# tanmaniac/IntroToComputerVision

Hardware: AMD Instinct MI355X
Metric: Mpix/s (LK 5-level pyramid, 1080p pairs) (higher is better)
Workload: dtype f32

## Files before the change

### introtocomputervision_amd/csrc/lk_fused.hip

```cpp
#include "lk_fused.hpp"

#include <cstdio>
#include <cstdlib>
#include <mutex>
#include <utility>
#include <vector>

#include "lk_device.hpp"
#include "lk_window.hpp"

namespace micv {



template <int NT, int V4, int NROWS>
__device__ __forceinline__ void dma_rows(const float *__restrict__ src, int istride, float *dst, int tid) {
    constexpr int NP = (NROWS * V4 + NT - 1) / NT, A = NT / V4, B = NT % V4;
    const int lane = tid & 63;
    const int slot0 = __builtin_amdgcn_readfirstlane(tid - lane);
    int ly = tid / V4, lv = tid - ly * V4;
    size_t goff = (size_t)ly * istride + 4 * lv;
    const size_t step = (size_t)A * istride + 4 * B, carry = (size_t)istride - 4 * V4;
#pragma unroll
    for (int k = 0; k < NP; k++) {
        if (k == NP - 1 ? (ly < NROWS) : true)
            __builtin_amdgcn_global_load_lds((glb_cvoid *)(src + goff), (lds_void *)(dst + 4 * (slot0 + k * NT)), 16,
                                             0, 0);
        if (k + 1 < NP) {
            lv += B;
            const bool c = lv >= V4;
            lv -= c ? V4 : 0;
            ly += A + (c ? 1 : 0);
            goff += step + (c ? carry : 0);
        }
    }
}

template <int NT, int V4, int NROWS, bool ZERO>
__device__ __forceinline__ void dma_rows_clipped(const float *__restrict__ img, int istride, int rows, int cols,
                                                 int gx0, int gy0, float *dst, int tid) {
    constexpr int NP = (NROWS * V4 + NT - 1) / NT, A = NT / V4, B = NT % V4;
    const int lane = tid & 63;
    const int slot0 = __builtin_amdgcn_readfirstlane(tid - lane);
    int ly = tid / V4, lv = tid - ly * V4;
#pragma unroll
    for (int k = 0; k < NP; k++) {
        if (k == NP - 1 ? (ly < NROWS) : true) {
            const int gy = gy0 + ly, gx = gx0 + 4 * lv;
            const bool in = (unsigned)gy < (unsigned)rows && (unsigned)gx < (unsigned)cols;
            if (in)
                __builtin_amdgcn_global_load_lds((glb_cvoid *)(img + (size_t)gy * istride + gx),
                                                 (lds_void *)(dst + 4 * (slot0 + k * NT)), 16, 0, 0);
            else if (ZERO)
                *reinterpret_cast<v4f *>(dst + 4 * (tid + k * NT)) = (v4f){0.f, 0.f, 0.f, 0.f};
        }
        if (k + 1 < NP) {
            lv += B;
            const bool c = lv >= V4;
            lv -= c ? V4 : 0;
            ly += A + (c ? 1 : 0);
        }
    }
}

template <int NT, int RWC, int NROWS>
__device__ __forceinline__ void dma_gather(const float *__restrict__ src, int rstride, int xs, float *dst, int tid) {
    constexpr int PARTS = (RWC + 63) / 64, NWV = NT / 64, RSTEP = NWV / PARTS, NP = (NROWS + RSTEP - 1) / RSTEP;
    static_assert(NWV % PARTS == 0 && RSTEP >= 1, "a wave keeps its part of the row");
    const int lane = tid & 63, wave = __builtin_amdgcn_readfirstlane(tid >> 6);
    const int part = wave % PARTS, col = 64 * part + lane;
    const unsigned voff = (unsigned)(col * xs);
    if (col < RWC) {
#pragma unroll
        for (int k = 0; k < NP; k++) {
            const int row = wave / PARTS + RSTEP * k;
            if (k == NP - 1 ? row < NROWS : true)
                __builtin_amdgcn_global_load_lds((glb_cvoid *)(src + (size_t)row * rstride + voff),
                                                 (lds_void *)(dst + row * RWC + 64 * part), 4, 0, 0);
        }
    }
}

template <int NT, int RWC, int NROWS, bool ZERO>
__device__ __forceinline__ void dma_gather_clipped(const float *__restrict__ img, int rstride, int xs, int rows,
                                                   int cols, int gx0, int gy0, float *dst, int tid) {
    constexpr int PARTS = (RWC + 63) / 64, NWV = NT / 64, RSTEP = NWV / PARTS, NP = (NROWS + RSTEP - 1) / RSTEP;
    static_assert(NWV % PARTS == 0 && RSTEP >= 1, "a wave keeps its part of the row");
    const int lane = tid & 63, wave = __builtin_amdgcn_readfirstlane(tid >> 6);
    const int part = wave % PARTS, col = 64 * part + lane;
    const int gx = gx0 + col;
    const bool col_in = (unsigned)gx < (unsigned)cols;
    const unsigned voff = col_in ? (unsigned)(gx * xs) : 0u;
    if (col < RWC) {
#pragma unroll
        for (int k = 0; k < NP; k++) {
            const int row = wave / PARTS + RSTEP * k;
            if (k == NP - 1 ? row < NROWS : true) {
                const int gy = gy0 + row;
                const bool row_in = (unsigned)gy < (unsigned)rows;
                if (row_in && col_in)
                    __builtin_amdgcn_global_load_lds((glb_cvoid *)(img + (size_t)gy * rstride + voff),
                                                     (lds_void *)(dst + row * RWC + 64 * part), 4, 0, 0);
                else if (ZERO)
                    dst[row * RWC + col] = 0.f;
            }
        }
    }
}

template <typename C>
__device__ __forceinline__ void dma_coarse(const LkLevelArgs &a, int pair, int cx0, int cy0, float *Cf, int tid) {
    constexpr int Q = C::CWP / 4, HPI = 64 / Q, HALF_ROWS = 2 * C::CH, NI = (HALF_ROWS + HPI - 1) / HPI;
    constexpr int NWV = C::NT / 64;
    const int lane = tid & 63, wave = __builtin_amdgcn_readfirstlane(tid >> 6);
    const int hl = lane / Q, q = lane - hl * Q;
    const int fc = a.flow_cols;
    const float *__restrict__ fu = a.flow_u + pair * a.flow_pair + (size_t)cy0 * fc + cx0 + 4 * q;
    const float *__restrict__ fv = a.flow_v + pair * a.flow_pair + (size_t)cy0 * fc + cx0 + 4 * q;
#pragma unroll
    for (int k = 0; k < (NI + NWV - 1) / NWV; k++) {
        const int it = wave + NWV * k;
        const int hr = it * HPI + hl;
        if (it < NI && hl < HPI && hr < HALF_ROWS)
            __builtin_amdgcn_global_load_lds((glb_cvoid *)(((hr & 1) ? fv : fu) + (size_t)(hr >> 1) * fc),
                                             (lds_void *)(Cf + it * HPI * C::CWP), 16, 0, 0);
    }
}

#include "lk_strip.hpp"

struct LkStreamLink {
    const int4 *sched;
    int per_xcd, xcd;
    unsigned *counter;
    int *slot;
    int4 next;
    bool next_staged;
    float ou[8], ov[8];
};

template <typename C>
__device__ __forceinline__ bool lk_tile_interior(const LkLevelArgs &a, int tile_x, int tile_y) {
    constexpr int E = C::M > 2 ? C::M : 2;
    const int rx0 = tile_x * C::TW - C::H, ry0 = tile_y * C::TH - C::H;
    return rx0 - E >= 0 && rx0 + C::RW + E <= a.cols && ry0 - E >= 0 && ry0 + C::RH + E <= a.rows;
}

template <typename C>
__device__ __forceinline__ void lk_stage_ahead(const LkLevelArgs &a, float *lds, int tile_x, int tile_y, int pair,
                                               int tid) {
    float *Xs = lds + C::IMG_F;
    const int rx0 = tile_x * C::TW - C::H, ry0 = tile_y * C::TH - C::H;
    const int cx0 = (rx0 - 2 > 0 ? rx0 - 2 : 0) >> 1, cy0 = (ry0 - 2 > 0 ? ry0 - 2 : 0) >> 1;
    dma_coarse<C>(a, pair, cx0, cy0, Xs, tid);
    const float *next = a.next + pair * a.img_pair;
    dma_rows<C::NT, C::NW / 4, C::NH>(next + (size_t)(ry0 - C::M) * a.img_stride + rx0 - C::M, a.img_stride,
                                      Xs + C::CS_F, tid);
}

template <int R, int MODE, bool INT, int NTV, bool CARRY = false, int THV = 32, bool STREAM = false,
          bool IN_LOOP = CARRY || STREAM, bool GATHER = false, bool PARTIAL_COLS = false, int TWV = 64, bool PRE = false>
__device__ __forceinline__ void lk_tile(const LkLevelArgs &a, const TapsN<2 * R + 1> &g,
                                        float *lds, int tile_x, int tile_y, int pair, bool more = false,
                                        LkStreamLink *link = nullptr) {
    using C = LkCfg<R, NTV, THV, TWV>;
    constexpr int RPT = C::RPT;
    constexpr int TW = C::TW, TH = C::TH, H = C::H, RW = C::RW, RH = C::RH, PS = C::PS;
    static_assert(TWV == 64 || (!CARRY && !STREAM && !GATHER), "32-wide tiles: the plain kernel only");
    constexpr int GW = C::GW, GH = C::GH, GS = C::GS, GP = C::GP, CW = C::CW, NT = C::NT;
    constexpr int M = C::M, NW = C::NW;
    static_assert(!CARRY || (INT && C::FAST && MODE == LK_FLOW_COARSE && C::CHAIN_OK), "carry tiles: interior, coarse flow");
    static_assert(!STREAM || (INT && C::FAST && MODE == LK_FLOW_COARSE && !CARRY && C::RW % 4 == 0 && C::NW % 4 == 0 && !GATHER),
                  "streamed tiles: interior, coarse flow, LDS-DMA staging");
    static_assert(!(STREAM || (INT && C::FAST && MODE == LK_FLOW_COARSE && !CARRY)) || C::CS_F + C::NW * C::NH <= C::X_F,
                  "interior tiles: DMA-staged coarse block + next window fit the gradient area");
    constexpr int LY0 = CARRY ? C::LYC : 0;
    constexpr int Q0 = CARRY ? C::QC : 0;
    constexpr int CH = CARRY ? C::CHC : C::CH;
    constexpr int NH = CARRY ? C::NHC : C::NH;
    constexpr bool CDMA = STREAM || (INT && C::FAST && MODE == LK_FLOW_COARSE && !CARRY);
    constexpr int CBF = CDMA ? C::CS_F : (CARRY ? C::CC_F : C::C_F);
    constexpr bool STAGED = INT && C::FAST && MODE != LK_FLOW_NONE;
#ifdef MICV_LK_DEFER_PREV
    constexpr bool DEFER = INT && C::FAST && MODE == LK_FLOW_COARSE && !CARRY && !STREAM && !GATHER;
#else
    constexpr bool DEFER = false;
#endif
    const bool fastb = !INT && C::FAST && MODE != LK_FLOW_NONE && a.rows >= 4 && a.cols >= 4;
    float *P = lds;
    float *Wp = lds + RH * PS;
    float *X = lds + C::IMG_F;
    float *Xs = X + (CARRY ? C::CARRY_F : 0);
    v2f *Cuv = reinterpret_cast<v2f *>(Xs);
    float *Ru = Xs + CBF, *Rv = Ru + CH * RW;
    float *Nx = Xs + CBF;
    float *Gx = X, *Gy = X + GP, *Gt = X + 2 * GP;
    float *rb0 = lds, *rb1 = lds + GH * C::RBS, *rb2 = lds + 2 * GH * C::RBS;

    int tid_ = threadIdx.x;
    if (IN_LOOP) asm volatile("" : "+v"(tid_));
    const int tid = tid_;
    const int rows = a.rows, cols = a.cols;
    const int x0 = tile_x * TW, y0 = tile_y * TH + a.y_shift;
    const int rx0 = x0 - H, ry0 = y0 - H;
    const float *__restrict__ prev = a.prev + pair * a.img_pair;
    const float *__restrict__ next = a.next + pair * a.img_pair;
    const int istride = a.img_stride;
    const int xs = GATHER ? a.img_xstride : 1;
    const float g5[5] = {0.0625f, 0.25f, 0.375f, 0.25f, 0.0625f};
#ifdef MICV_DIAG
    const bool stamp_wave = a.stamps != nullptr && __builtin_amdgcn_readfirstlane(tid) < 64;
    unsigned long long t_prev = 0;
    if (stamp_wave) t_prev = __builtin_amdgcn_s_memtime();
#define MICV_STAMP(k)                                                        \
    if (stamp_wave) {                                                        \
        const unsigned long long t_now = __builtin_amdgcn_s_memtime();       \
        if (tid == 0) atomicAdd(&a.stamps[(k) + (INT ? 0 : 8)], t_now - t_prev); \
        t_prev = t_now;                                                      \
    }                                                                        \
    if (a.stop_after == (k)) return;
#define MICV_STOP(k) if (a.stop_after == (k)) return;
#else
#define MICV_STAMP(k)
#define MICV_STOP(k)
#endif

    int cx0 = 0, cy0 = 0;
    constexpr int NC = CDMA ? 1 : (CH * CW + NT - 1) / NT;
    float rcu[NC], rcv[NC];
    if (CDMA) {
        cx0 = (rx0 - 2 > 0 ? rx0 - 2 : 0) >> 1;
        cy0 = (ry0 - 2 > 0 ? ry0 - 2 : 0) >> 1;
        if (!STREAM) dma_coarse<C>(a, pair, cx0, cy0, Xs, tid);
    } else if (MODE == LK_FLOW_COARSE) {
        const float *__restrict__ fu = a.flow_u + pair * a.flow_pair;
        const float *__restrict__ fv = a.flow_v + pair * a.flow_pair;
        const int fr = a.flow_rows, fc = a.flow_cols;
        cx0 = (rx0 - 2 > 0 ? rx0 - 2 : 0) >> 1;
        cy0 = (ry0 + (CARRY ? H : 0) - 2 > 0 ? ry0 + (CARRY ? H : 0) - 2 : 0) >> 1;
        if (fastb) {
            cx0 = (rx0 - 2) >> 1;
            cy0 = (ry0 - 2) >> 1;
        }
#pragma unroll
        for (int k = 0; k < NC; k++) {
            const int i = tid + k * NT < CH * CW ? tid + k * NT : CH * CW - 1;
            const int cy = i / CW, cx = i - cy * CW;
            const int yy = clampi(cy0 + cy, 0, fr - 1), xx = clampi(cx0 + cx, 0, fc - 1);
            rcu[k] = fu[(size_t)yy * fc + xx];
            rcv[k] = fv[(size_t)yy * fc + xx];
        }
    }
    const bool vec_ok = STREAM || GATHER ||
                        (INT && (istride & 3) == 0 && ((a.img_pair & 3) == 0) &&
                         ((reinterpret_cast<uintptr_t>(a.prev) | reinterpret_cast<uintptr_t>(a.next)) & 15) == 0);
    constexpr bool DMA_OK = (RW % 4 == 0) && (NW % 4 == 0);
    bool deferred = false;
    if (INT && DMA_OK && vec_ok) {
        constexpr int V = RW / 4;
        if constexpr (GATHER) {
            if (STAGED)
                dma_gather<NT, NW, NH>(next + (ptrdiff_t)(ry0 - M + LY0) * istride + (ptrdiff_t)(rx0 - M) * xs, istride, xs, Nx, tid);
            dma_gather<NT, RW, RH - LY0>(prev + (size_t)(ry0 + LY0) * istride + (size_t)rx0 * xs, istride, xs, P + LY0 * RW, tid);
            if (MODE == LK_FLOW_NONE)
                dma_gather<NT, RW, RH - LY0>(next + (size_t)(ry0 + LY0) * istride + (size_t)rx0 * xs, istride, xs, Wp + LY0 * RW, tid);
        } else if constexpr (DEFER) {
            dma_rows<NT, NW / 4, NH>(next + (size_t)(ry0 - M + LY0) * istride + rx0 - M, istride, Nx, tid);
            dma_rows<NT, V, RH - LY0>(prev + (size_t)(ry0 + LY0) * istride + rx0, istride, P + LY0 * RW, tid);
            deferred = true;
        } else {
        dma_rows<NT, V, RH - LY0>(prev + (size_t)(ry0 + LY0) * istride + rx0, istride, P + LY0 * RW, tid);
        if (MODE == LK_FLOW_NONE)
            dma_rows<NT, V, RH - LY0>(next + (size_t)(ry0 + LY0) * istride + rx0, istride, Wp + LY0 * RW, tid);
        if (STAGED && !STREAM)
            dma_rows<NT, NW / 4, NH>(next + (size_t)(ry0 - M + LY0) * istride + rx0 - M, istride, Nx, tid);
        }
        if (MODE == LK_FLOW_COARSE && !CDMA) {
#pragma unroll
            for (int k = 0; k < NC; k++) {
                const int i = tid + k * NT;
                if (i < CH * CW) {
                    Cuv[i] = (v2f){rcu[k], rcv[k]};
                }
            }
        }
    } else {
        if (MODE == LK_FLOW_COARSE && !CDMA) {
#pragma unroll
            for (int k = 0; k < NC; k++) {
                const int i = tid + k * NT;
                if (i < CH * CW) {
                    Cuv[i] = (v2f){rcu[k], rcv[k]};
                }
            }
        }
        const bool clip_dma = fastb && (GATHER || ((cols & 3) == 0 && (istride & 3) == 0 && ((a.img_pair & 3) == 0) &&
                              ((reinterpret_cast<uintptr_t>(a.prev) | reinterpret_cast<uintptr_t>(a.next)) & 15) == 0));
        if (GATHER && clip_dma) {
            dma_gather_clipped<NT, NW, NH, true>(next, istride, xs, rows, cols, rx0 - M, ry0 - M, Nx, tid);
            dma_gather_clipped<NT, RW, RH, false>(prev, istride, xs, rows, cols, rx0, ry0, P, tid);
        } else if (clip_dma) {
            dma_rows_clipped<NT, RW / 4, RH, false>(prev, istride, rows, cols, rx0, ry0, P, tid);
            dma_rows_clipped<NT, NW / 4, NH, true>(next, istride, rows, cols, rx0 - M, ry0 - M, Nx, tid);
        } else
        {
            constexpr int NB = (RH * RW + NT - 1) / NT;
            float rp[NB], rn[NB];
#pragma unroll
            for (int k = 0; k < NB; k++) {
                const int i = tid + k * NT < RH * RW ? tid + k * NT : RH * RW - 1;
                const int ly = i / RW, lx = i - ly * RW;
                const int gy = clampi(ry0 + ly, 0, rows - 1), gx = clampi(rx0 + lx, 0, cols - 1);
                rp[k] = prev[(size_t)gy * istride + (size_t)gx * xs];
                if (MODE == LK_FLOW_NONE) rn[k] = next[(size_t)gy * istride + (size_t)gx * xs];
            }
#pragma unroll
            for (int k = 0; k < NB; k++) {
                const int i = tid + k * NT;
                if (i < RH * RW) {
                    P[i] = rp[k];
                    if (MODE == LK_FLOW_NONE) Wp[i] = rn[k];
                }
            }
        }
        if (STAGED) {
            for (int i = tid; i < NH * NW; i += NT) {
                const int ly = i / NW, lx = i - ly * NW;
                Nx[i] = next[(ptrdiff_t)(ry0 - M + LY0 + ly) * istride + (ptrdiff_t)(rx0 - M + lx) * xs];
            }
        }
        if (fastb && !clip_dma) {
            constexpr int NBN = (NH * NW + NT - 1) / NT, HB = (NBN + 1) / 2, A = NT / NW, B = NT % NW;
            int ly = tid / NW, lx = tid - ly * NW;
#pragma unroll
            for (int half = 0; half < 2; half++) {
                float rn[HB];
                int ly2 = ly, lx2 = lx;
#pragma unroll
                for (int k = 0; k < HB; k++) {
                    const int gy = ry0 - M + ly2, gx = rx0 - M + lx2;
                    const bool ok = (unsigned)gy < (unsigned)rows && (unsigned)gx < (unsigned)cols;
                    const float val = next[(size_t)clampi(gy, 0, rows - 1) * istride + (size_t)clampi(gx, 0, cols - 1) * xs];
                    rn[k] = ok ? val : 0.f;
                    lx2 += B;
                    const bool c = lx2 >= NW;
                    lx2 -= c ? NW : 0;
                    ly2 += A + (c ? 1 : 0);
                }
#pragma unroll
                for (int k = 0; k < HB; k++) {
                    const int i = tid + (half * HB + k) * NT;
                    if (i < NH * NW) Nx[i] = rn[k];
                }
                ly = ly2;
                lx = lx2;
            }
        }
    }
    float base_u[RPT], base_v[RPT];
#pragma unroll
    for (int j = 0; j < RPT; j++) base_u[j] = base_v[j] = 0.f;
    if (MODE == LK_FLOW_NONE && a.base_rmw) {
        const int c_ = threadIdx.x & (TW - 1), r0_ = RPT * (threadIdx.x / TW);
#pragma unroll
        for (int j = 0; j < RPT; j++) {
            const int gy = y0 + r0_ + j, gx = x0 + c_;
            if (gy < rows && gx < cols) {
                base_u[j] = a.out_u[pair * a.out_pair + (size_t)gy * a.out_stride + gx];
                base_v[j] = a.out_v[pair * a.out_pair + (size_t)gy * a.out_stride + gx];
            }
        }
    }
    if constexpr (DEFER) {
        if (deferred) {
            constexpr int V = RW / 4, TOT = (RH - LY0) * V, NPP = (TOT + NT - 1) / NT;
            static_assert(NPP >= 1 && NPP <= 8, "prev transfers per wave");
            const bool last = __builtin_amdgcn_readfirstlane(tid) + (NPP - 1) * NT < TOT;
            if (last) {
                asm volatile("s_waitcnt vmcnt(%0)" ::"n"(NPP) : "memory");
            } else {
                asm volatile("s_waitcnt vmcnt(%0)" ::"n"(NPP - 1) : "memory");
            }
            __builtin_amdgcn_s_barrier();
            asm volatile("" ::: "memory");
        } else {
            __syncthreads();
        }
    } else if (MODE != LK_FLOW_NONE && !STREAM) __syncthreads();
    MICV_STAMP(0)

    if (MODE != LK_FLOW_NONE) {
        if (C::FAST && (INT || fastb)) {
            int nx0s = rx0 - M, ny0s = ry0 - M + LY0;
            asm("" : "+s"(nx0s), "+s"(ny0s));
            auto march = [&](int lx, int ly0, float *bu8, float *bv8) {
                const int gx = rx0 + lx, gy0 = ry0 + ly0;
                const float xf32 = 32.f * (float)gx, yf32 = 32.f * (float)gy0;
                typedef __attribute__((address_space(3))) float lds_float;
                lds_float *wrow = (lds_float *)(Wp + ly0 * PS + lx);
                asm("" : "+v"(wrow));
                v2f ruv[RPT / 2 + 2];
                if (MODE == LK_FLOW_COARSE) {
                    const int cyb = ((gy0 >> 1) - 1) - cy0;
                    const int ccb = ((gx >> 1) - 1) - cx0;
                    const int odd = gx & 1;
                    const bool first_col = !INT && gx == 0, last_col = !INT && gx == cols - 1;
                    constexpr int NR = RPT / 2 + 2;
                    v2f cc[CDMA ? 5 * NR : 1];
                    if constexpr (CDMA)
                        coarse_block_load<C>(cc, Xs + cyb * (2 * C::CWP) + ccb, odd, std::make_integer_sequence<int, NR>{});
#pragma unroll
                    for (int i = 0; i < NR; i++) {
                        v2f c0, c1, c2, ca, cb;
                        if constexpr (CDMA) {
                            c0 = cc[5 * i], c1 = cc[5 * i + 1], c2 = cc[5 * i + 2], ca = cc[5 * i + 3], cb = cc[5 * i + 4];
                        } else {
                            const v2f *c = Cuv + (cyb + i) * CW + ccb;
                            c0 = c[0];
                            c1 = c[1];
                            c2 = c[2];
                            ca = c[odd];
                            cb = c[1 + odd];
                        }
                        const v2f t0 = first_col ? c2 : c0, t4 = last_col ? c0 : c2;
                        v2f t = t0 * (v2f){g5[0], g5[0]};
                        t = __builtin_elementwise_fma(ca, (v2f){g5[1], g5[1]}, t);
                        t = __builtin_elementwise_fma(c1, (v2f){g5[2], g5[2]}, t);
                        t = __builtin_elementwise_fma(cb, (v2f){g5[3], g5[3]}, t);
                        ruv[i] = __builtin_elementwise_fma(t4, (v2f){g5[4], g5[4]}, t);
                    }
                }
                float fu_[RPT], fv_[RPT];
                if (MODE == LK_FLOW_FULL) {
#pragma unroll
                    for (int j = 0; j < RPT; j++) {
                        const size_t fo = pair * a.flow_pair + (size_t)(INT ? gy0 + j : clampi(gy0 + j, 0, rows - 1)) * a.flow_cols +
                                          (INT ? gx : clampi(gx, 0, cols - 1));
                        fu_[j] = a.flow_u[fo];
                        fv_[j] = a.flow_v[fo];
                    }
                }
#pragma unroll
                for (int p = 0; p < RPT / 2; p++) {
#pragma unroll
                    for (int o = 0; o < 2; o++) {
                        const int j = 2 * p + o;
                        float bu, bv;
                        v2f half_uv;
                        if (MODE == LK_FLOW_COARSE) {
                            const int i1 = o ? p + 1 : p, i3 = o ? p + 2 : p + 1;
                            v2f ra = ruv[p], rc = ruv[p + 2];
                            if (!INT) asm("" : "+v"(ra), "+v"(rc));
                            const v2f r0 = (!INT && gy0 + j == 0) ? rc : ra;
                            const v2f r4 = (!INT && gy0 + j == rows - 1) ? ra : rc;
                            v2f auv = r0 * (v2f){g5[0], g5[0]};
                            auv = __builtin_elementwise_fma(ruv[i1], (v2f){g5[1], g5[1]}, auv);
                            auv = __builtin_elementwise_fma(ruv[p + 1], (v2f){g5[2], g5[2]}, auv);
                            auv = __builtin_elementwise_fma(ruv[i3], (v2f){g5[3], g5[3]}, auv);
                            auv = __builtin_elementwise_fma(r4, (v2f){g5[4], g5[4]}, auv);
                            half_uv = auv;
                            auv = auv * (v2f){2.f, 2.f};
                            bu = auv.x;
                            bv = auv.y;
                        } else {
                            bu = fu_[j];
                            bv = fv_[j];
                            half_uv = (v2f){bu, bv};
                        }
                        bu8[j] = bu;
                        bv8[j] = bv;
                        if constexpr (DEFER) {
                            if (deferred) {
                                const float wv = warp_sample_staged<NW, NH, 64, true>(
                                    Nx, nx0s, ny0s, next, rows, cols, istride, (v2f){xf32, yf32 + 32.f * (float)j}, half_uv, xs);
                                asm volatile("ds_write_b32 %0, %1 offset:%2" ::"v"(wrow), "v"(wv), "n"(4 * j * PS) : "memory");
                            } else {
                                wrow[j * PS] = warp_sample_staged<NW, NH, 64>(
                                    Nx, nx0s, ny0s, next, rows, cols, istride, (v2f){xf32, yf32 + 32.f * (float)j}, half_uv, xs);
                            }
                        } else if (!CARRY || ly0 + j >= LY0)
                            wrow[j * PS] = warp_sample_staged<NW, NH, MODE == LK_FLOW_COARSE ? 64 : 32>(
                                Nx, nx0s, ny0s, next, rows, cols, istride, (v2f){xf32, yf32 + 32.f * (float)j}, half_uv, xs);
                        if (NT >= 512) __builtin_amdgcn_sched_barrier(0);
                    }
                }
            };
            march(H + (tid & (TW - 1)), H + RPT * (tid / TW), base_u, base_v);
            constexpr int BS = H / RPT, NB = CARRY ? BS : 2 * BS;
            constexpr int SEG0 = CARRY ? (LY0 - H) / RPT : 0, NJ = NB * RW + 2 * H * (TH / RPT - SEG0);
            static_assert(!CARRY || (LY0 >= H && LY0 < H + TH), "carry rows start inside the tile's own rows");
            for (int n = tid; n < (PRE && a.pre_warp ? 0 : NJ); n += NT) {
                int lx, ly0;
                if (n < NB * RW) {
                    const int band = n / RW + (CARRY ? BS : 0);
                    lx = n - (band - (CARRY ? BS : 0)) * RW;
                    ly0 = band < BS ? band * RPT : H + TH + (band - BS) * RPT;
                } else {
                    const int m = n - NB * RW;
                    const int seg = m / (2 * H) + SEG0, cc = m - (seg - SEG0) * (2 * H);
                    lx = cc < H ? cc : TW + cc;
                    ly0 = H + RPT * seg;
                }
                float tu[RPT], tv[RPT];
                march(lx, ly0, tu, tv);
            }
        } else {
            if (MODE == LK_FLOW_COARSE) {
                const int fr = a.flow_rows;
                for (int i = tid; i < CH * RW; i += NT) {
                    const int cy = i / RW, lx = i - cy * RW;
                    const int gx = rx0 + lx;
                    if ((INT || (unsigned)gx < (unsigned)cols) && cy0 + cy < fr) {
                        float au = 0.f, av = 0.f;
#pragma unroll
                        for (int k = 0; k < 5; k++) {
                            const int sc = ((INT ? gx + k - 2 : reflect101(gx + k - 2, cols)) >> 1) - cx0;
                            const v2f cuv = Cuv[cy * CW + sc];
                            au = fmaf(cuv.x, g5[k], au);
                            av = fmaf(cuv.y, g5[k], av);
                        }
                        Ru[i] = au;
                        Rv[i] = av;
                    }
                }
                __syncthreads();
                MICV_STAMP(1)
            }
            auto do_px = [&](int ly, int lx, float &bu, float &bv) {
                const int gy = ry0 + ly, gx = rx0 + lx;
                if (!INT && ((unsigned)gy >= (unsigned)rows || (unsigned)gx >= (unsigned)cols)) return;
                if (MODE == LK_FLOW_COARSE) {
                    float au = 0.f, av = 0.f;
#pragma unroll
                    for (int k = 0; k < 5; k++) {
                        const int rr = ((INT ? gy + k - 2 : reflect101(gy + k - 2, rows)) >> 1) - cy0;
                        au = fmaf(Ru[rr * RW + lx], g5[k], au);
                        av = fmaf(Rv[rr * RW + lx], g5[k], av);
                    }
                    bu = au * 2.f;
                    bv = av * 2.f;
                } else {
                    bu = a.flow_u[pair * a.flow_pair + (size_t)gy * a.flow_cols + gx];
                    bv = a.flow_v[pair * a.flow_pair + (size_t)gy * a.flow_cols + gx];
                }
                Wp[ly * PS + lx] = warp_sample(next, rows, cols, istride, gx, gy, bu, bv, xs);
            };
            {
                const int c = tid & (TW - 1), grp = tid / TW;
#pragma unroll
                for (int j = 0; j < RPT; j++) do_px(H + RPT * grp + j, H + c, base_u[j], base_v[j]);
            }
            constexpr int NHALO = 2 * H * RW + TH * 2 * H;
            for (int n = tid; n < NHALO; n += NT) {
                int ly, lx;
                if (n < 2 * H * RW) {
                    ly = n / RW;
                    lx = n - ly * RW;
                    if (ly >= H) ly += TH;
                } else {
                    const int m = n - 2 * H * RW;
                    const int rr = m / (2 * H), cc = m - rr * (2 * H);
                    ly = H + rr;
                    lx = cc < H ? cc : TW + cc;
                }
                float du_, dv_;
                do_px(ly, lx, du_, dv_);
            }
        }
    }
    if constexpr (DEFER) {
        if (deferred) asm volatile("s_waitcnt vmcnt(0) lgkmcnt(0)" ::: "memory");
    }
    __syncthreads();
    MICV_STAMP(2)
    if constexpr (PRE) {
        if (a.pre_warp) {
            const int c = tid & (TW - 1), r0 = RPT * (tid / TW);
            const int gx = x0 + c;
            float *__restrict__ wb = a.grad + pair * a.grad_pair;
            float *__restrict__ ou = a.out_u + pair * a.out_pair;
            float *__restrict__ ov = a.out_v + pair * a.out_pair;
            if (INT || gx < cols) {
#pragma unroll
                for (int j = 0; j < RPT; j++) {
                    const int gy = y0 + r0 + j;
                    if (INT || gy < rows) {
                        wb[(size_t)gy * cols + gx] = Wp[(H + r0 + j) * PS + H + c];
                        ou[(size_t)gy * a.out_stride + gx] = base_u[j];
                        ov[(size_t)gy * a.out_stride + gx] = base_v[j];
                    }
                }
            }
            return;
        }
    }
    int ticket = 0;
    if (STREAM && tid == 0) ticket = (int)atomicAdd(link->counter, 1u);

    {
        const float s1 = 1.f / 9.f, s2 = 2.f * s1;
        if (!INT) {
            for (int n = tid; n < 2 * RW + 2 * RH; n += NT) {
                int ly, lx;
                if (n < 2 * RW) {
                    ly = (n < RW ? -1 : rows) - ry0;
                    lx = n < RW ? n : n - RW;
                } else {
                    const int m = n - 2 * RW;
                    lx = (m < RH ? -1 : cols) - rx0;
                    ly = m < RH ? m : m - RH;
                }
                if ((unsigned)ly >= (unsigned)RH || (unsigned)lx >= (unsigned)RW) continue;
                const int gy = ry0 + ly, gx = rx0 + lx;
                if (gy >= -1 && gy <= rows && gx >= -1 && gx <= cols) {
                    const int sy = reflect101(gy, rows) - ry0, sx = reflect101(gx, cols) - rx0;
                    if ((unsigned)sy < (unsigned)RH && (unsigned)sx < (unsigned)RW) {
                        P[ly * PS + lx] = P[sy * PS + sx];
                        Wp[ly * PS + lx] = Wp[sy * PS + sx];
                    }
                }
            }
            __syncthreads();
        }
        {
            constexpr int SEG = CARRY ? 6 : (TH == 16 ? 5 : (NT >= 512 ? 4 : 16)), NSEG = (GH - Q0 + SEG - 1) / SEG;
            static_assert(GW % 2 == 0, "gradient columns in pairs");
            constexpr int GW2 = GW / 2;
            const v2f s1v = {s1, s1}, s2v = {s2, s2}, halfv = {0.5f, 0.5f};
            for (int n = tid; n < GW2 * NSEG; n += NT) {
                const int seg = n / GW2, qx = 2 * (n - seg * GW2);
                const int q0 = Q0 + seg * SEG, q1 = q0 + SEG < GH ? q0 + SEG : GH;
                const int lx = qx + (H - R);
                v2f ptx[3], pty[3], wtx[3], wty[3], pcc[3], wcc[3];
                auto rowpass = [&](int ly, int slot) {
                    const float *pr = P + ly * PS + lx, *wr = Wp + ly * PS + lx;
                    v2f pa, pb, pc, wa, wb, wc;
                    if constexpr (((H - R) & 1) == 1 && (PS & 1) == 0) {
                        const v2f p01 = *reinterpret_cast<const v2f *>(pr - 1), p23 = *reinterpret_cast<const v2f *>(pr + 1);
                        const v2f w01 = *reinterpret_cast<const v2f *>(wr - 1), w23 = *reinterpret_cast<const v2f *>(wr + 1);
                        pa = p01; pb = (v2f){p01.y, p23.x}; pc = p23;
                        wa = w01; wb = (v2f){w01.y, w23.x}; wc = w23;
                    } else {
                        pa = (v2f){pr[-1], pr[0]}; pb = (v2f){pr[0], pr[1]}; pc = (v2f){pr[1], pr[2]};
                        wa = (v2f){wr[-1], wr[0]}; wb = (v2f){wr[0], wr[1]}; wc = (v2f){wr[1], wr[2]};
                    }
                    ptx[slot] = pc - pa;
                    pty[slot] = __builtin_elementwise_fma(pc, s1v, __builtin_elementwise_fma(pb, s2v, pa * s1v));
                    wtx[slot] = wc - wa;
                    wty[slot] = __builtin_elementwise_fma(wc, s1v, __builtin_elementwise_fma(wb, s2v, wa * s1v));
                    pcc[slot] = pb;
                    wcc[slot] = wb;
                };
                const int lyb = q0 + (H - R);
                rowpass(lyb - 1, 0);
                rowpass(lyb, 1);
                constexpr int TRIP = SEG <= 6 ? SEG : 3;
#pragma unroll 1
                for (int qy = q0; qy < q1; qy += TRIP) {
#pragma unroll
                    for (int t = 0; t < TRIP; t++) {
                        if (qy + t < q1) {
                            const int s_new = (t + 2) % 3, s_top = t % 3, s_mid = (t + 1) % 3;
                            rowpass(qy + t + (H - R) + 1, s_new);
                            const v2f pgx = __builtin_elementwise_fma(
                                ptx[s_new], s1v, __builtin_elementwise_fma(ptx[s_mid], s2v, ptx[s_top] * s1v));
                            const v2f pgy = pty[s_new] - pty[s_top];
                            const v2f ngx = __builtin_elementwise_fma(
                                wtx[s_new], s1v, __builtin_elementwise_fma(wtx[s_mid], s2v, wtx[s_top] * s1v));
                            const v2f ngy = wty[s_new] - wty[s_top];
                            *reinterpret_cast<v2f *>(Gx + (qy + t) * GS + qx) = ngx * halfv + pgx * halfv;
                            *reinterpret_cast<v2f *>(Gy + (qy + t) * GS + qx) = ngy * halfv + pgy * halfv;
                            *reinterpret_cast<v2f *>(Gt + (qy + t) * GS + qx) = wcc[s_mid] - pcc[s_mid];
                        }
                    }
                }
            }
        }
        if (!INT) {
            __syncthreads();
            auto fill = [&](int qy, int qx) {
                const int gy = y0 - R + qy, gx = x0 - R + qx;
                const int sy = reflect101(gy, rows) - (y0 - R), sx = reflect101(gx, cols) - (x0 - R);
                const bool ok = (unsigned)sy < (unsigned)GH && (unsigned)sx < (unsigned)GW;
                Gx[qy * GS + qx] = ok ? Gx[sy * GS + sx] : 0.f;
                Gy[qy * GS + qx] = ok ? Gy[sy * GS + sx] : 0.f;
                Gt[qy * GS + qx] = ok ? Gt[sy * GS + sx] : 0.f;
            };
            const int rt = clampi(-(y0 - R), 0, GH), rb = clampi(rows - (y0 - R), rt, GH);
            const int cl = clampi(-(x0 - R), 0, GW), cr = clampi(cols - (x0 - R), cl, GW);
            const int n_full = (rt + GH - rb) * GW, side = cl + GW - cr;
            for (int i = tid; i < n_full; i += NT) {
                const int r = i / GW, qx = i - r * GW;
                fill(r < rt ? r : rb + (r - rt), qx);
            }
            if (side > 0) {
                for (int i = tid; i < (rb - rt) * 16; i += NT) {
                    const int qy = rt + (i >> 4);
                    for (int cc = i & 15; cc < side; cc += 16) fill(qy, cc < cl ? cc : cr + (cc - cl));
                }
            }
        }
    }
    __syncthreads();
    MICV_STAMP(3)

    if constexpr (PRE) {
        static_assert(MODE == LK_FLOW_COARSE && !CARRY && !STREAM && TWV == 64, "pre-pass tiles: coarse flow, plain launch");
        const int c = tid & (TW - 1), r0 = RPT * (tid / TW);
        const int gx = x0 + c, pad = a.grad_pad, gp = a.grad_pitch;
        const size_t rowp = 3 * (size_t)gp;
        float *__restrict__ gb = a.grad + pair * a.grad_pair;
        float *__restrict__ ou = a.out_u + pair * a.out_pair;
        float *__restrict__ ov = a.out_v + pair * a.out_pair;
        if (INT || gx < cols) {
            int px2 = -1;
            if (!INT) {
                if (gx >= 1 && gx <= pad) px2 = pad - gx;
                else if (gx >= cols - 1 - pad && gx <= cols - 2) px2 = pad + 2 * (cols - 1) - gx;
            }
#pragma unroll
            for (int j = 0; j < RPT; j++) {
                const int gy = y0 + r0 + j;
                if (INT || gy < rows) {
                    const int q = r0 + j + R, qx = c + R;
                    const float ix = Gx[q * GS + qx], iy = Gy[q * GS + qx], it = Gt[q * GS + qx];
                    auto put = [&](int py, int px) {
                        float *d = gb + (size_t)py * rowp + px;
                        d[0] = ix;
                        d[gp] = iy;
                        d[2 * gp] = it;
                    };
                    put(gy + pad, gx + pad);
                    if (!INT) {
                        int py2 = -1;
                        if (gy >= 1 && gy <= pad) py2 = pad - gy;
                        else if (gy >= rows - 1 - pad && gy <= rows - 2) py2 = pad + 2 * (rows - 1) - gy;
                        if (py2 >= 0) put(py2, gx + pad);
                        if (px2 >= 0) put(gy + pad, px2);
                        if (py2 >= 0 && px2 >= 0) put(py2, px2);
                    }
                    if (a.pre_base) {
                        ou[(size_t)gy * a.out_stride + gx] = base_u[j];
                        ov[(size_t)gy * a.out_stride + gx] = base_v[j];
                    }
                }
            }
        }
        return;
    }

    const int c = tid & (TW - 1), r0 = RPT * (tid / TW);
    float Sxx[RPT], Sxy[RPT], Syy[RPT], Sxt[RPT], Syt[RPT];
    constexpr int RPW = 64 / (TW / 4);
    constexpr int RPI = RPW * (NT / 64);
    constexpr int SWEEP_UNROLL = NT >= 512 ? 1 : 4;
    constexpr int SWEEP_TRIPS = (GH + RPI - 1) / RPI;
    const int sweep_trips = SWEEP_TRIPS == 1 ? 1 + (a.batch < 0 ? 1 : 0) : SWEEP_TRIPS;
    {
        const int lane = tid & 63, wave = tid >> 6;
        const int grp = TW == 64 ? lane >> 2 : ((lane & 3) | ((lane >> 2) & 4)), c0 = 4 * grp;
        const int lrow = TW == 64 ? (lane & 3) : (((lane >> 2) & 3) | ((lane >> 3) & 4));
#pragma unroll SWEEP_UNROLL
        for (int it = 0; it < sweep_trips; it++) {
            const int qy = it * RPI + wave * RPW + lrow;
            if (qy < GH) {
                v2f wx[2 * C::WV], wy[2 * C::WV];
                load_window_pairs<C>(Gx, qy, c0, wx);
                load_window_pairs<C>(Gy, qy, c0, wy);
                const int o = TW == 64 ? rb_off(qy, grp) : rb_off32(qy, grp);
                row_taps_skew<C>(wx, wx, g, rb0 + o);
                if (TH == 16) __builtin_amdgcn_sched_barrier(0);
                row_taps_skew<C>(wx, wy, g, rb1 + o);
                if (TH == 16) __builtin_amdgcn_sched_barrier(0);
                row_taps_skew<C>(wy, wy, g, rb2 + o);
            }
        }
        if (STREAM && tid == 0) *link->slot = ticket;
        __syncthreads();
        MICV_STOP(41)
        int cls[TW == 64 ? 4 : 8];
        if constexpr (TW == 64) {
            col_bases<C>(rb0, c, r0, cls);
            col_pass<C, 0, PARTIAL_COLS>(cls, Sxx, g);
            col_pass<C, 1, PARTIAL_COLS>(cls, Sxy, g);
            col_pass<C, 2, PARTIAL_COLS>(cls, Syy, g);
        } else {
            col_bases32<C>(rb0, c, r0, cls);
            col_pass32<C, 0, PARTIAL_COLS>(cls, Sxx, g);
            col_pass32<C, 1, PARTIAL_COLS>(cls, Sxy, g);
            col_pass32<C, 2, PARTIAL_COLS>(cls, Syy, g);
        }
        if (TH == 16) __builtin_amdgcn_sched_barrier(0);
        __syncthreads();
        MICV_STOP(42)
#pragma unroll SWEEP_UNROLL
        for (int it = 0; it < sweep_trips; it++) {
            const int qy = it * RPI + wave * RPW + lrow;
            if (qy < GH) {
                v2f wx[2 * C::WV], wt[2 * C::WV];
                load_window_pairs<C>(Gx, qy, c0, wx);
                load_window_pairs<C>(Gt, qy, c0, wt);
                const int o = TW == 64 ? rb_off(qy, grp) : rb_off32(qy, grp);
                row_taps_skew<C>(wx, wt, g, rb0 + o);
                if (NT >= 512) __builtin_amdgcn_sched_barrier(0);
                load_window_pairs<C>(Gy, qy, c0, wx);
                row_taps_skew<C>(wx, wt, g, rb1 + o);
            }
        }
        __syncthreads();
        MICV_STOP(43)
        if constexpr (STREAM) {
            const int t = __builtin_amdgcn_readfirstlane(*link->slot);
            link->next = make_int4(0, 0, 0, 0);
            link->next_staged = false;
            if (t < link->per_xcd) {
                const int4 e2 = link->sched[8 * t + link->xcd];
                link->next = e2;
                if (e2.z > 0 && lk_tile_interior<C>(a, e2.x, e2.y)) {
                    lk_stage_ahead<C>(a, lds, e2.x, e2.y, e2.w, tid);
                    link->next_staged = true;
                }
            }
        }
        if (INT && C::CHAIN_OK && MODE == LK_FLOW_COARSE && more) {
            const v4f *src = reinterpret_cast<const v4f *>(X + TH * GS);
            v4f *dst = reinterpret_cast<v4f *>(X);
            for (int i = tid; i < C::CARRY_F / 4; i += NT) dst[i] = src[i];
        }
        if constexpr (TW == 64) {
            col_pass<C, 0, PARTIAL_COLS>(cls, Sxt, g);
            col_pass<C, 1, PARTIAL_COLS>(cls, Syt, g);
        } else {
            col_pass32<C, 0, PARTIAL_COLS>(cls, Sxt, g);
            col_pass32<C, 1, PARTIAL_COLS>(cls, Syt, g);
        }
    }
    MICV_STAMP(4)

    float *__restrict__ ou = a.out_u + pair * a.out_pair;
    float *__restrict__ ov = a.out_v + pair * a.out_pair;
    const int gx = x0 + c;
    if (INT || gx < cols) {
#pragma unroll
        for (int j = 0; j < RPT; j++) {
            const int gy = y0 + r0 + j;
            if (gy >= a.row_begin && gy < a.row_end) {
                float uu, vv;
                lk_solve(Sxx[j], Sxy[j], Syy[j], Sxt[j], Syt[j], uu, vv);
                if (a.add_base) {
                    uu = base_u[j] + uu;
                    vv = base_v[j] + vv;
                }
                if constexpr (STREAM) {
                    link->ou[j] = uu;
                    link->ov[j] = vv;
                } else {
                    ou[(size_t)gy * a.out_stride + gx] = uu;
                    ov[(size_t)gy * a.out_stride + gx] = vv;
                }
            }
        }
    }
    MICV_STAMP(5)
#undef MICV_STAMP
#undef MICV_STOP
}

template <typename C>
__device__ __forceinline__ void lk_tile_of(const LkLevelArgs &a, int bidx, int &tile_x, int &tile_y) {
    constexpr int E = C::M > 2 ? C::M : 2;
    const int nb = gridDim.x, per = nb >> 3, rem = nb & 7;
    const int xcd = bidx & 7, idx = bidx >> 3;
    const int tiles_x = (a.cols + C::TW - 1) / C::TW;
    const int tiles_y = nb / tiles_x, ty_base = a.row_begin / C::TH;
    {
        constexpr int FX = C::TW + C::H + E, FY = C::TH + C::H + E;
        int ix0 = (C::H + E + C::TW - 1) / C::TW, ix1 = a.cols >= FX ? (a.cols - FX) / C::TW + 1 : 0;
        int iy0 = (C::H + E - a.y_shift + C::TH - 1) / C::TH - ty_base;
        int iy1 = (a.rows >= FY + a.y_shift ? (a.rows - FY - a.y_shift) / C::TH + 1 : 0) - ty_base;
        ix1 = ix1 < tiles_x ? ix1 : tiles_x;
        iy0 = iy0 > 0 ? iy0 : 0;
        iy1 = iy1 < tiles_y ? iy1 : tiles_y;
        const int iw = ix1 > ix0 ? ix1 - ix0 : 0, ih = iy1 > iy0 ? iy1 - iy0 : 0;
        const int ni = iw * ih, nbd = nb - ni;
        const int t_plain = xcd * per + (xcd < rem ? xcd : rem) + idx;
        if (ni * 2 >= nb && nb >= 64) {
            const int b0 = (int)(((long long)xcd * nbd) >> 3), b1 = (int)(((long long)(xcd + 1) * nbd) >> 3);
            if (idx < b1 - b0) {
                int b = b0 + idx;
                const int n_top = iy0 * tiles_x, n_bot = (tiles_y - iy1) * tiles_x, side = tiles_x - iw;
                if (b < n_top) {
                    tile_y = b / tiles_x;
                    tile_x = b - tile_y * tiles_x;
                } else if (b < n_top + n_bot) {
                    b -= n_top;
                    tile_y = b / tiles_x;
                    tile_x = b - tile_y * tiles_x;
                    tile_y += iy1;
                } else {
                    b -= n_top + n_bot;
                    const int r = b / side, c = b - r * side;
                    tile_y = iy0 + r;
                    tile_x = c < ix0 ? c : c + iw;
                }
            } else {
                const int i = t_plain - b1;
                const int r = i / iw;
                tile_y = iy0 + r;
                tile_x = ix0 + (i - r * iw);
            }
        } else {
            tile_y = t_plain / tiles_x;
            tile_x = t_plain - tile_y * tiles_x;
        }
        tile_y += ty_base;
    }
}

template <int NT>
__device__ __forceinline__ void lk_build_block(const LkBuildJob &j, int block, int tid) {
    constexpr int RPT = 32 / (NT / 64);
    static_assert(NT % 64 == 0 && 32 % (NT / 64) == 0, "a unit is 32 rows x 64 lanes");
    const int lane = tid & 63, trow = (tid >> 6) * RPT;
    const int l = j.level, rl = j.rows >> l, cl = j.cols >> l;
    const int bx = l == 1 ? (cl + 127) / 128 : (cl + 63) / 64, per_img = bx * ((rl + 31) / 32);
    for (int u = block; u < j.units; u += j.blocks) {
        const int img = u / per_img, r = u - img * per_img;
        const int set = img / j.batch, b = img - set * j.batch;
        const int byi = r / bx, bxi = r - byi * bx;
        const int y0 = byi * 32 + trow;
        const float *src = (set ? j.src_b : j.src_a) + b * j.img_elems;
        float *dst = (set ? j.pyr_b : j.pyr_a) + j.dst_off + (size_t)b * rl * cl;
        if (l == 1) {
            const int x2 = bxi * 64 + lane;
            if (2 * x2 >= cl) continue;
            float4 q[RPT];
#pragma unroll
            for (int i = 0; i < RPT; i++)
                if (y0 + i < rl) q[i] = *reinterpret_cast<const float4 *>(src + (size_t)(2 * (y0 + i) + 1) * j.sstride + 4 * x2);
#pragma unroll
            for (int i = 0; i < RPT; i++)
                if (y0 + i < rl) *reinterpret_cast<float2 *>(dst + (size_t)(y0 + i) * cl + 2 * x2) = make_float2(q[i].y, q[i].w);
        } else {
            const int x = bxi * 64 + lane, sh = (1 << l) - 1;
            if (x >= cl) continue;
            float q[RPT];
#pragma unroll
            for (int i = 0; i < RPT; i++)
                if (y0 + i < rl) q[i] = src[(size_t)(((y0 + i) << l) + sh) * j.sstride + (x << l) + sh];
#pragma unroll
            for (int i = 0; i < RPT; i++)
                if (y0 + i < rl) dst[(size_t)(y0 + i) * cl + x] = q[i];
        }
    }
}

template <int R, int MODE, int NTV, int THV = 32, bool GATHER = false, int TWV = 64>
__global__ __launch_bounds__(NTV, lk_waves_per_simd_rt(R, NTV, THV)) void lk_level_kernel(LkLevelArgs a, TapsN<2 * R + 1> g) {
    using C = LkCfg<R, NTV, THV, TWV>;
    extern __shared__ __attribute__((aligned(16))) float lds[];
    constexpr int E = C::M > 2 ? C::M : 2;
    if (blockIdx.y >= a.batch) {
        lk_build_block<NTV>(a.job, (blockIdx.y - a.batch) * gridDim.x + blockIdx.x, threadIdx.x);
        return;
    }
    int tile_x, tile_y;
    lk_tile_of<C>(a, blockIdx.x, tile_x, tile_y);
    const int rx0 = tile_x * C::TW - C::H, ry0 = tile_y * C::TH + a.y_shift - C::H;
    const bool interior = rx0 - E >= 0 && rx0 + C::RW + E <= a.cols && ry0 - E >= 0 &&
                          ry0 + C::RH + E <= a.rows;
    if (interior)
        lk_tile<R, MODE, true, NTV, false, THV, false, false, GATHER, true, TWV>(a, g, lds, tile_x, tile_y, blockIdx.y);
    else
        lk_tile<R, MODE, false, NTV, false, THV, false, false, GATHER, true, TWV>(a, g, lds, tile_x, tile_y, blockIdx.y);
}

template <int R, int NTV, int THV = 32>
__global__ __launch_bounds__(NTV, lk_waves_per_simd(NTV)) void lk_grad_kernel(LkLevelArgs a) {
    using C = LkCfg<R, NTV, THV>;
    extern __shared__ __attribute__((aligned(16))) float lds[];
    constexpr int E = C::M > 2 ? C::M : 2;
    int tile_x, tile_y;
    lk_tile_of<C>(a, blockIdx.x, tile_x, tile_y);
    const int rx0 = tile_x * C::TW - C::H, ry0 = tile_y * C::TH - C::H;
    const bool interior = rx0 - E >= 0 && rx0 + C::RW + E <= a.cols && ry0 - E >= 0 && ry0 + C::RH + E <= a.rows;
    TapsN<2 * R + 1> g = {};
    if (interior)
        lk_tile<R, LK_FLOW_COARSE, true, NTV, false, THV, false, false, false, false, 64, true>(a, g, lds, tile_x, tile_y, blockIdx.y);
    else
        lk_tile<R, LK_FLOW_COARSE, false, NTV, false, THV, false, false, false, false, 64, true>(a, g, lds, tile_x, tile_y, blockIdx.y);
}

struct LkStripPlan {
    int items, strips, segs, seg_rows;
    int ix0, iw, iy0, ih;
    int tiles_x, tiles_y, border;
};

template <int R, int NTV>
__global__ __launch_bounds__(NTV, lk_waves_per_simd(NTV)) void lk_level_strip_kernel(LkLevelArgs a, TapsN<2 * R + 1> g, LkStripPlan p) {
    using C = LkCfg<R, NTV>;
    extern __shared__ __attribute__((aligned(16))) float lds[];
    int b = blockIdx.x;
    if (b < p.items) {
        const int per = p.items >> 3, rem = p.items & 7;
        const int xcd = b & 7, idx = b >> 3;
        int item = xcd * per + (xcd < rem ? xcd : rem) + idx;
        if (idx >= per + (xcd < rem ? 1 : 0)) return;
        const int strip = item % p.strips, t = item / p.strips;
        const int seg = t % p.segs, pair = t / p.segs;
        const int x0 = (p.ix0 + strip) * C::TW;
        const int s0 = p.iy0 * C::TH + seg * p.seg_rows;
        const int end = (p.iy0 + p.ih) * C::TH;
        const int s1 = s0 + p.seg_rows < end ? s0 + p.seg_rows : end;
        lk_strip<R>(a, g, lds, x0, s0, s1, pair);
        return;
    }
    b -= p.items;
    const int pair = b / p.border;
    b -= pair * p.border;
    int tile_x, tile_y;
    const int iy1 = p.iy0 + p.ih, n_top = p.iy0 * p.tiles_x, n_bot = (p.tiles_y - iy1) * p.tiles_x, side = p.tiles_x - p.iw;
    if (b < n_top) {
        tile_y = b / p.tiles_x;
        tile_x = b - tile_y * p.tiles_x;
    } else if (b < n_top + n_bot) {
        b -= n_top;
        tile_y = b / p.tiles_x;
        tile_x = b - tile_y * p.tiles_x;
        tile_y += iy1;
    } else {
        b -= n_top + n_bot;
        const int r = b / side, c = b - r * side;
        tile_y = p.iy0 + r;
        tile_x = c < p.ix0 ? c : c + p.iw;
    }
    lk_tile<R, LK_FLOW_COARSE, false, NTV>(a, g, lds, tile_x, tile_y, pair);
}

template <int R, int NTV, bool GATHER = false>
__global__ __launch_bounds__(NTV, lk_waves_per_simd(NTV)) void lk_level_chain_kernel(LkLevelArgs a, TapsN<2 * R + 1> g,
                                                                        const int4 *__restrict__ sched) {
    using C = LkCfg<R, NTV>;
    extern __shared__ __attribute__((aligned(16))) float lds[];
    constexpr int E = C::M > 2 ? C::M : 2;
    if (a.job.blocks && (int)blockIdx.x >= a.job.first_block) {
        lk_build_block<NTV>(a.job, blockIdx.x - a.job.first_block, threadIdx.x);
        return;
    }
    const int4 e = sched[blockIdx.x];
    if (e.z <= 0) return;
    const int rx0 = e.x * C::TW - C::H, ry0 = e.y * C::TH - C::H;
    const bool interior = rx0 - E >= 0 && rx0 + C::RW + E <= a.cols && ry0 - E >= 0 &&
                          ry0 + C::RH + E <= a.rows;
    if (!interior) {
        lk_tile<R, LK_FLOW_COARSE, false, NTV, false, 32, false, false, GATHER>(a, g, lds, e.x, e.y, e.w);
        return;
    }
    lk_tile<R, LK_FLOW_COARSE, true, NTV, false, 32, false, false, GATHER>(a, g, lds, e.x, e.y, e.w, e.z > 1);
    for (int t = 1; t < e.z; t++) {
        __syncthreads();
        lk_tile<R, LK_FLOW_COARSE, true, NTV, true, 32, false, true, GATHER>(a, g, lds, e.x, e.y + t, e.w, t + 1 < e.z);
    }
}

template <int R, int NTV, int THV = 32>
__global__ __launch_bounds__(NTV, lk_waves_per_simd(NTV)) void lk_level_stream_kernel(LkLevelArgs a, TapsN<2 * R + 1> g,
                                                                         const int4 *__restrict__ sched, int per_xcd,
                                                                         unsigned *__restrict__ tickets) {
    using C = LkCfg<R, NTV, THV>;
    extern __shared__ __attribute__((aligned(16))) float lds[];
    __shared__ int slot;
    const int tid = threadIdx.x;
    LkStreamLink link;
    link.sched = sched;
    link.per_xcd = per_xcd;
    link.xcd = blockIdx.x & 7;
    link.counter = tickets + link.xcd;
    link.slot = &slot;
    link.next = make_int4(0, 0, 0, 0);
    link.next_staged = false;
    if (tid == 0) slot = (int)atomicAdd(link.counter, 1u);
    __syncthreads();
    int t = __builtin_amdgcn_readfirstlane(slot);
    int4 e = t < per_xcd ? sched[8 * t + link.xcd] : make_int4(0, 0, 0, 0);
    bool staged = false;
    int4 pending = make_int4(0, 0, 0, 0);
    auto flush = [&]() {
        if (pending.z > 0) {
            float *__restrict__ ou = a.out_u + pending.w * a.out_pair;
            float *__restrict__ ov = a.out_v + pending.w * a.out_pair;
            const int gx = pending.x * C::TW + (tid & (C::TW - 1));
            const int gy0 = pending.y * C::TH + C::RPT * (tid / C::TW);
#pragma unroll
            for (int j = 0; j < C::RPT; j++) {
                ou[(size_t)(gy0 + j) * a.out_stride + gx] = link.ou[j];
                ov[(size_t)(gy0 + j) * a.out_stride + gx] = link.ov[j];
            }
            pending.z = 0;
        }
    };
    while (e.z > 0) {
        if (lk_tile_interior<C>(a, e.x, e.y)) {
            if (!staged) {
                lk_stage_ahead<C>(a, lds, e.x, e.y, e.w, tid);
                __syncthreads();
            }
            flush();
            lk_tile<R, LK_FLOW_COARSE, true, NTV, false, THV, true>(a, g, lds, e.x, e.y, e.w, false, &link);
            pending = e;
            e = link.next;
            staged = link.next_staged;
        } else {
            flush();
            int tk = 0;
            if (tid == 0) tk = (int)atomicAdd(link.counter, 1u);
            lk_tile<R, LK_FLOW_COARSE, false, NTV, false, THV, false, true>(a, g, lds, e.x, e.y, e.w);
            if (tid == 0) slot = tk;
            __syncthreads();
            t = __builtin_amdgcn_readfirstlane(slot);
            e = t < per_xcd ? sched[8 * t + link.xcd] : make_int4(0, 0, 0, 0);
            staged = false;
        }
        __syncthreads();
    }
    flush();
    if (tid == 0) {
        __threadfence();
        if (atomicAdd(tickets + 8, 1u) == gridDim.x - 1) {
            for (int x = 0; x < 8; x++) tickets[x] = 0;
            tickets[8] = 0;
            __threadfence();
        }
    }
// ... 418 lines not shown
```

Baseline: 57380.

## Skip out-of-image warping, gradient and window work in boundary tiles

For non-interior (boundary) tiles, precomputes the tile's valid row and column extents. It then skips warp sampling for positions outside the image, gradient segments outside the valid range, row sweeps past the last output row, and column passes for waves whose rows are all beyond row_end. The coarse-flow store is moved after the clipped DMA so it can overlap with the loads. Only edge tiles benefit, so the overall effect depends on what fraction of tiles are boundary tiles across the pyramid levels. The changes add extra branches and risk leaving stale LDS values wherever later code still reads skipped regions.

```diff
diff --git a/introtocomputervision_amd/csrc/lk_fused.hip b/introtocomputervision_amd/csrc/lk_fused.hip
--- a/introtocomputervision_amd/csrc/lk_fused.hip
+++ b/introtocomputervision_amd/csrc/lk_fused.hip
@@ -203,6 +203,19 @@
     const int rows = a.rows, cols = a.cols;
     const int x0 = tile_x * TW, y0 = tile_y * TH + a.y_shift;
     const int rx0 = x0 - H, ry0 = y0 - H;
+    int lt = 0, lb = RH, ll = 0, lr = RW, ye = TH, qe = GH, rt = 0, rb = GH, cl = 0, cr = GW;
+    if constexpr (!INT) {
+        lt = clampi(-ry0, 0, RH);
+        lb = clampi(rows - ry0, lt, RH);
+        ll = clampi(-rx0, 0, RW);
+        lr = clampi(cols - rx0, ll, RW);
+        ye = clampi(a.row_end - y0, 0, TH);
+        qe = ye + 2 * R;
+        rt = clampi(-(y0 - R), 0, GH);
+        rb = clampi(rows - (y0 - R), rt, GH);
+        cl = clampi(-(x0 - R), 0, GW);
+        cr = clampi(cols - (x0 - R), cl, GW);
+    }
     const float *__restrict__ prev = a.prev + pair * a.img_pair;
     const float *__restrict__ next = a.next + pair * a.img_pair;
     const int istride = a.img_stride;
@@ -285,23 +298,28 @@
             }
         }
     } else {
-        if (MODE == LK_FLOW_COARSE && !CDMA) {
-#pragma unroll
-            for (int k = 0; k < NC; k++) {
-                const int i = tid + k * NT;
-                if (i < CH * CW) {
-                    Cuv[i] = (v2f){rcu[k], rcv[k]};
-                }
-            }
-        }
         const bool clip_dma = fastb && (GATHER || ((cols & 3) == 0 && (istride & 3) == 0 && ((a.img_pair & 3) == 0) &&
                               ((reinterpret_cast<uintptr_t>(a.prev) | reinterpret_cast<uintptr_t>(a.next)) & 15) == 0));
+        auto store_coarse = [&]() {
+            if (MODE == LK_FLOW_COARSE && !CDMA) {
+#pragma unroll
+                for (int k = 0; k < NC; k++) {
+                    const int i = tid + k * NT;
+                    if (i < CH * CW) {
+                        Cuv[i] = (v2f){rcu[k], rcv[k]};
+                    }
+                }
+            }
+        };
+        if (INT || !clip_dma) store_coarse();
         if (GATHER && clip_dma) {
             dma_gather_clipped<NT, NW, NH, true>(next, istride, xs, rows, cols, rx0 - M, ry0 - M, Nx, tid);
             dma_gather_clipped<NT, RW, RH, false>(prev, istride, xs, rows, cols, rx0, ry0, P, tid);
+            if constexpr (!INT) store_coarse();
         } else if (clip_dma) {
             dma_rows_clipped<NT, RW / 4, RH, false>(prev, istride, rows, cols, rx0, ry0, P, tid);
             dma_rows_clipped<NT, NW / 4, NH, true>(next, istride, rows, cols, rx0 - M, ry0 - M, Nx, tid);
+            if constexpr (!INT) store_coarse();
         } else
         {
             constexpr int NB = (RH * RW + NT - 1) / NT;
@@ -485,7 +503,9 @@
                     }
                 }
             };
-            march(H + (tid & (TW - 1)), H + RPT * (tid / TW), base_u, base_v);
+            auto in_image = [&](int lx, int ly0) { return INT || (ly0 < lb && ly0 + RPT > lt && lx < lr && lx >= ll); };
+            if (in_image(H + (tid & (TW - 1)), H + RPT * (tid / TW)))
+                march(H + (tid & (TW - 1)), H + RPT * (tid / TW), base_u, base_v);
             constexpr int BS = H / RPT, NB = CARRY ? BS : 2 * BS;
             constexpr int SEG0 = CARRY ? (LY0 - H) / RPT : 0, NJ = NB * RW + 2 * H * (TH / RPT - SEG0);
             static_assert(!CARRY || (LY0 >= H && LY0 < H + TH), "carry rows start inside the tile's own rows");
@@ -502,7 +522,7 @@
                     ly0 = H + RPT * seg;
                 }
                 float tu[RPT], tv[RPT];
-                march(lx, ly0, tu, tv);
+                if (in_image(lx, ly0)) march(lx, ly0, tu, tv);
             }
         } else {
             if (MODE == LK_FLOW_COARSE) {
@@ -631,6 +651,7 @@
                 const int seg = n / GW2, qx = 2 * (n - seg * GW2);
                 const int q0 = Q0 + seg * SEG, q1 = q0 + SEG < GH ? q0 + SEG : GH;
                 const int lx = qx + (H - R);
+                if (!INT && (q0 >= (rb < qe ? rb : qe) || q1 <= rt || qx >= cr || qx + 2 <= cl)) continue;
                 v2f ptx[3], pty[3], wtx[3], wty[3], pcc[3], wcc[3];
                 auto rowpass = [&](int ly, int slot) {
                     const float *pr = P + ly * PS + lx, *wr = Wp + ly * PS + lx;
@@ -686,15 +707,13 @@
                 Gy[qy * GS + qx] = ok ? Gy[sy * GS + sx] : 0.f;
                 Gt[qy * GS + qx] = ok ? Gt[sy * GS + sx] : 0.f;
             };
-            const int rt = clampi(-(y0 - R), 0, GH), rb = clampi(rows - (y0 - R), rt, GH);
-            const int cl = clampi(-(x0 - R), 0, GW), cr = clampi(cols - (x0 - R), cl, GW);
-            const int n_full = (rt + GH - rb) * GW, side = cl + GW - cr;
+            const int n_full = (rt + (qe > rb ? qe - rb : 0)) * GW, side = cl + GW - cr;
             for (int i = tid; i < n_full; i += NT) {
                 const int r = i / GW, qx = i - r * GW;
                 fill(r < rt ? r : rb + (r - rt), qx);
             }
             if (side > 0) {
-                for (int i = tid; i < (rb - rt) * 16; i += NT) {
+                for (int i = tid; i < ((rb < qe ? rb : qe) - rt) * 16; i += NT) {
                     const int qy = rt + (i >> 4);
                     for (int cc = i & 15; cc < side; cc += 16) fill(qy, cc < cl ? cc : cr + (cc - cl));
                 }
@@ -763,7 +782,7 @@
 #pragma unroll SWEEP_UNROLL
         for (int it = 0; it < sweep_trips; it++) {
             const int qy = it * RPI + wave * RPW + lrow;
-            if (qy < GH) {
+            if (qy < qe) {
                 v2f wx[2 * C::WV], wy[2 * C::WV];
                 load_window_pairs<C>(Gx, qy, c0, wx);
                 load_window_pairs<C>(Gy, qy, c0, wy);
@@ -779,11 +798,14 @@
         __syncthreads();
         MICV_STOP(41)
         int cls[TW == 64 ? 4 : 8];
+        const bool live = INT || TW != 64 || __builtin_amdgcn_readfirstlane(r0) < ye;
         if constexpr (TW == 64) {
             col_bases<C>(rb0, c, r0, cls);
-            col_pass<C, 0, PARTIAL_COLS>(cls, Sxx, g);
-            col_pass<C, 1, PARTIAL_COLS>(cls, Sxy, g);
-            col_pass<C, 2, PARTIAL_COLS>(cls, Syy, g);
+            if (live) {
+                col_pass<C, 0, PARTIAL_COLS>(cls, Sxx, g);
+                col_pass<C, 1, PARTIAL_COLS>(cls, Sxy, g);
+                col_pass<C, 2, PARTIAL_COLS>(cls, Syy, g);
+            }
         } else {
             col_bases32<C>(rb0, c, r0, cls);
             col_pass32<C, 0, PARTIAL_COLS>(cls, Sxx, g);
@@ -796,7 +818,7 @@
 #pragma unroll SWEEP_UNROLL
         for (int it = 0; it < sweep_trips; it++) {
             const int qy = it * RPI + wave * RPW + lrow;
-            if (qy < GH) {
+            if (qy < qe) {
                 v2f wx[2 * C::WV], wt[2 * C::WV];
                 load_window_pairs<C>(Gx, qy, c0, wx);
                 load_window_pairs<C>(Gt, qy, c0, wt);
@@ -828,8 +850,10 @@
             for (int i = tid; i < C::CARRY_F / 4; i += NT) dst[i] = src[i];
         }
         if constexpr (TW == 64) {
-            col_pass<C, 0, PARTIAL_COLS>(cls, Sxt, g);
-            col_pass<C, 1, PARTIAL_COLS>(cls, Syt, g);
+            if (live) {
+                col_pass<C, 0, PARTIAL_COLS>(cls, Sxt, g);
+                col_pass<C, 1, PARTIAL_COLS>(cls, Syt, g);
+            }
         } else {
             col_pass32<C, 0, PARTIAL_COLS>(cls, Sxt, g);
             col_pass32<C, 1, PARTIAL_COLS>(cls, Syt, g);
```

Result: no change. 57780, median of 6 (+0.7%).
